# charleschen003/doudizhu-rl

Measured on AMD Instinct MI355X. Metric: env steps/sec (batched tables), higher is better.
Workload: dtype u8; 1 GPU; 65536 tables per GPU, random policy (engine RNG), legal-move list only (no NN), auto-reset: the workload of BASELINE.json configs[1] at the largest single-GPU table count (65,536 per GPU: configs[2] / configs[3]; configs[4] = 8 x 65,536), the same per-GPU workload at every N; tables_per_gpu=65536, total_tables=65536, episodes=2767981, list_layout=slab (fixed-stride segment per table)

## Files before the change

doudizhu-rl_amd/csrc/ddz_engine.hip:

```cpp
#include <hip/hip_runtime.h>
#include <stddef.h>
#include <stdint.h>
#include <stdlib.h>
#include <string.h>

#include <atomic>
#include <mutex>

#include "../../include/ddz_env.h"
#include "ddz_device.h"

using namespace ddz;

namespace {

constexpr int BLOCK = 256;
constexpr int WPB = 16;
constexpr int TB = WPB * 64;
constexpr int STATE_ROW_BYTES = DDZ_NFIELDS * DDZ_ROW;

constexpr int F_ENUM = 1, F_STEP = 2, F_RESET = 4, F_COUNT = 8, F_SLAB = 16;

constexpr int AUTO_SLOTS = 4;
constexpr int AO_HDR_BYTES = 576;
// ... 193 lines not shown
      if (legal) {
        const int64_t pos = o.base + n + pre;
        if (pos < o.cap) {
          o.rows[pos] = row;
          if (IDS) o.ids[pos] = id;
        }
      }
      if (EM == EM_PICK) {
        const int w = pk.want - n;
        if (w >= 0 && w < k) {
          const int src = __builtin_ctzll(__ballot(legal && pre == w));
          pk.r0 = rl(row.x, src); pk.r1 = rl(row.y, src); pk.r2 = rl(row.z, src); pk.r3 = rl(row.w, src);
        }
      }
    }
  }
  return n + k;
}

template <int EM, bool IDS, bool LEAD, class HT>
__device__ __forceinline__ int scan_ids(int id0, int count, const HT& hot, uint64_t hand8, const Follow& f,
                                        int lane, const Out& o, int n, Pick& pk) {
  constexpr bool ROWS = EM == EM_WRITE || EM == EM_PICK;
  constexpr uint64_t H8 = 0x8888888888888888ull;
  const int slot0 = id0 == ID_BIGBANG ? HOT_IDS : id0;
  if (EM == EM_TEAM_PLAN) {
    for (int j0 = 0; j0 < count; j0 += 64, ++pk.rc)
      if (pk.rc < TEAM_ROUNDS)
        pk.desc[pk.rc] = make_uint2(team_x(count - j0, id0 + j0, slot0 + j0), 0u);
    return n;
  }
  for (int j0 = 0; j0 < count; j0 += 64) {
    const int j = j0 + lane;
    const bool in = j < count;
    const int jj = in ? j : 0, id = id0 + jj;
    const uint4 m = hot.meta[slot0 + jj];
    static_assert(!ROWS || HT::HAS_ROWS, "this emission mode reads the unpacked rows");
    const uint4 row = ROWS ? hot.rows[HT::HAS_ROWS ? slot0 + jj : 0] : make_uint4(0, 0, 0, 0);
    const uint64_t nib = (uint64_t)m.x | ((uint64_t)m.y << 32);
    const bool sub = ((hand8 - nib) & H8) == H8;
    const int val = m.z & 0xFF, len = (m.z >> 8) & 0xFF, cat = (m.z >> 16) & 0xFF;
    const bool gate = LEAD || id == 0 || cat == BIGBANG || (cat == QUADRIC && (f.lc != QUADRIC || val > f.lv)) ||
                      (cat == f.lc && f.lc != QUADRIC && len == f.ll && val > f.lv);
    n = scan_emit<EM, IDS>(in && sub && gate, id, nib, cat, (int)(m.z & 0xFFFF), row, o, n, pk);
  }
  return n;
}

template <int EM, bool IDS, class HT>
__device__ __forceinline__ int scan_combos(int list, int count, int idb, uint64_t mainnib, int s, int gap, int mult,
                                           int cat, const HT& hot, uint64_t hand8, int lane, const Out& o,
                                           int n, Pick& pk) {
  constexpr bool ROWS = EM == EM_WRITE || EM == EM_PICK;
  constexpr uint64_t H8 = 0x8888888888888888ull;
  const int L = CL_L[list], off = CL_OFF[list];
  if (EM == EM_TEAM_PLAN) {
    for (int j0 = 0; j0 < count; j0 += 64, ++pk.rc)
      if (pk.rc < TEAM_ROUNDS)
        pk.desc[pk.rc] = make_uint2(team_x(count - j0, idb + j0, off + j0),
                                    1u | (uint32_t)L << 2 | (uint32_t)s << 5 | (uint32_t)gap << 9 | (uint32_t)mult << 12 | (uint32_t)cat << 14);
    return n;
  }
  for (int j0 = 0; j0 < count; j0 += 64) {
    const int j = j0 + lane;
    const bool in = j < count;
    uint64_t nib = mainnib;
    if constexpr (HT::HAS_C64) {
      const uint64_t c = hot.c64[off + (in ? j : 0)], lowm = (1ull << (4 * s)) - 1ull;
      nib += ((c & lowm) | ((c & ~lowm) << (4 * gap))) << (mult - 1);
    } else {
      const uint32_t e = hot.combo[off + (in ? j : 0)];
      for (int k = 0; k < L; ++k) {
        const int pos = (e >> (4 * k)) & 15;
        nib += (uint64_t)mult << (4 * (pos < s ? pos : pos + gap));
      }
    }
    const bool sub = ((hand8 - nib) & H8) == H8;
    const uint4 row = ROWS ? unpack_row(nib, (uint32_t)cat) : make_uint4(0, 0, 0, 0);
    n = scan_emit<EM, IDS>(in && sub, idb + j, nib, cat, s | (gap << 8), row, o, n, pk);
  }
  return n;
}

template <int EM, bool IDS, bool LEAD, class HT>
__device__ __forceinline__ int plan_scan_t(uint64_t hand, const Follow& f, const HT& hot, int lane, const Out& o, Pick& pk) {
  constexpr bool PRUNE = EM != EM_STAGE;
  const uint64_t hand8 = hand | 0x8888888888888888ull;
  const int cnt = lane < 15 ? (int)((hand >> (4 * (lane & 15))) & 15) : 0;
  const uint32_t m1 = (uint32_t)__ballot(cnt >= 1) & M15;
  const uint32_t m2 = (uint32_t)__ballot(cnt >= 2) & M13;
  const uint32_t m3 = (uint32_t)__ballot(cnt >= 3) & M13;
  const uint32_t m4 = (uint32_t)__ballot(cnt >= 4) & M13;
  int n = 0;
  auto scan = [&](int id0, int count) { n = scan_ids<EM, IDS, LEAD>(id0, count, hot, hand8, f, lane, o, n, pk); };
  if (!LEAD && f.lc == BIGBANG) {
    scan(0, 1);
    return n;
  }
  if (LEAD) scan(1, 54); else scan(0, 55);
  const uint32_t above = LEAD ? M15 : gt_mask(f.lv);
  if (LEAD || f.lc == THREE_ONE || f.lc == THREE_TWO) {
    const uint32_t mains = m3 & above;
    if (mains) {
      const int lo = __builtin_ctz(mains), hi = 31 - __builtin_clz(mains);
      if (LEAD || f.lc == THREE_ONE) scan(ID_THREE_ONE + 14 * lo, 14 * (hi - lo + 1));
      if ((LEAD || f.lc == THREE_TWO) && (!PRUNE || __builtin_popcount(m2) >= 2))
        scan(ID_THREE_TWO + 12 * lo, 12 * (hi - lo + 1));
    }
  }
  if (LEAD) {
    const bool a = run_starts(m1 & M12, 5) != 0, b = run_starts(m2 & M12, 3) != 0, c = run_starts(m3 & M12, 2) != 0;
    if (a || b || c) {
      const int lo = a ? ID_SINGLE_LINE : b ? ID_DOUBLE_LINE : ID_TRIPLE_LINE;
      const int hi = c ? ID_THREE_ONE_LINE : b ? ID_TRIPLE_LINE : ID_DOUBLE_LINE;
      scan(lo, hi - lo);
    }
  } else if (f.lc == SINGLE_LINE) {
    scan(ID_SINGLE_LINE, 36);
  } else if (f.lc == DOUBLE_LINE) {
    scan(ID_DOUBLE_LINE, 52);
  } else if (f.lc == TRIPLE_LINE) {
    scan(ID_TRIPLE_LINE, 45);
  }
  auto planes = [&](int cat, int hi, int idb0, int mult, int list2, int list3, int list4, int list5) {
    const uint32_t mm = m3 & M12;
    if (!(LEAD || f.lc == cat)) return;
    for (uint32_t st = mm & (mm >> 1); st; st &= st - 1) {
      const int s = __builtin_ctz(st);
      const int runlen = __builtin_ctz(~(mm >> s));
      int before, sz2, sz3, sz4;
      if (cat == THREE_ONE_LINE) {
        before = 879 * (s < 8 ? s : 8) + (s > 8 ? 627 : 0) + (s > 9 ? 297 : 0);
        sz2 = 77; sz3 = 220; sz4 = 330;
      } else {
        before = 301 * (s < 9 ? s : 9) + (s > 9 ? 175 : 0);
        sz2 = 55; sz3 = 120; sz4 = 126;
      }
      const int maxL = runlen < hi ? runlen : hi;
      for (int L = 2; L <= maxL && s + L <= 12; ++L) {
        if (!(LEAD || (L == f.ll && s > f.lv))) continue;
        if (PRUNE && __builtin_popcount((mult == 1 ? m1 : m2) & ~(((1u << L) - 1u) << s)) < L) continue;
        const int idb = idb0 + before + (L > 2 ? sz2 : 0) + (L > 3 ? sz3 : 0) + (L > 4 ? sz4 : 0);
        const int size = L == 2 ? sz2 : L == 3 ? sz3 : L == 4 ? sz4 : 252;
        const int list = L == 2 ? list2 : L == 3 ? list3 : L == 4 ? list4 : list5;
        const uint64_t mainnib = ((3ull * ONES) & ((1ull << (4 * L)) - 1ull)) << (4 * s);
        n = scan_combos<EM, IDS>(list, size, idb, mainnib, s, L, mult, cat, hot, hand8, lane, o, n, pk);
      }
    }
  };
  planes(THREE_ONE_LINE, 5, ID_THREE_ONE_LINE, 1, 1, 4, 6, 8);
  planes(THREE_TWO_LINE, 4, ID_THREE_TWO_LINE, 2, 3, 5, 7, 7);
  if ((m1 & JOKERS) == JOKERS) scan(ID_BIGBANG, 1);
  if (LEAD || f.lc == FOUR_TAKE_ONE)
    for (uint32_t qm = m4 & above; qm; qm &= qm - 1) {
      const int q = __builtin_ctz(qm);
      n = scan_combos<EM, IDS>(0, 90, ID_FOUR_TAKE_ONE + 90 * q, 4ull << (4 * q), q, 1, 1, FOUR_TAKE_ONE, hot, hand8,
                               lane, o, n, pk);
    }
  if (LEAD || f.lc == FOUR_TAKE_TWO)
    for (uint32_t qm = m4 & above; qm; qm &= qm - 1) {
      const int q = __builtin_ctz(qm);
      if (PRUNE && __builtin_popcount(m2 & ~(1u << q)) < 2) continue;
      n = scan_combos<EM, IDS>(2, 66, ID_FOUR_TAKE_TWO + 66 * q, 4ull << (4 * q), q, 1, 2, FOUR_TAKE_TWO, hot, hand8,
                               lane, o, n, pk);
    }
#if DDZ_NATIVE_JOKER_KICKERS
  if ((m1 & JOKERS) == JOKERS) {
    const uint32_t mm = m3 & M12;
    const uint32_t quads = (LEAD || f.lc == FOUR_TAKE_ONE) ? (m4 & above) : 0u;
    const uint32_t pairs3 = (LEAD || (f.lc == THREE_ONE_LINE && f.ll == 2)) ? (mm & (mm >> 1) & above) : 0u;
    if (EM == EM_TEAM_PLAN) {
      if (quads | pairs3) {
        if (pk.rc < TEAM_ROUNDS) pk.desc[pk.rc] = make_uint2(team_x(24, ID_JK_FOUR, 0), 2u | quads << 2 | pairs3 << 15);
        ++pk.rc;
      }
    } else if (quads | pairs3) {
      const bool isq = lane < 13;
      const int r = isq ? lane : (lane - 13) & 15;
      const bool ok = isq ? ((quads >> r) & 1u) : (lane < 24 && ((pairs3 >> r) & 1u));
      const uint64_t jk = (1ull << 52) | (1ull << 56);
      const uint64_t nib = (isq ? (4ull << (4 * r)) : (0x33ull << (4 * r))) | jk;
      const int cat = isq ? FOUR_TAKE_ONE : THREE_ONE_LINE;
// ... 337 lines not shown
    }
    if (RESET) {
      const uint8_t* mask = (const uint8_t*)a.sel;
      if (!mask || mask[t]) {
        changed = true;
        episode = dealt ? episode + 1 : 0;
        uint64_t h0, h1, h2;
        deal_wave(gid, episode, a.k0, a.k1, lane, h0, h1, h2);
        R = lane == 0 ? unpack_row(h0, 17) : lane == 1 ? unpack_row(h1, 20) : lane == 2 ? unpack_row(h2, 17)
            : lane == DDZ_F_META ? make_uint4(1u | (0xFFu << 16), 1u << 16, episode, 0) : make_uint4(0, 0, 0, 0);
        role = 1; is_done = false; dealt = true;
        qhand = h1; qinfo = mk_info(EMPTY, 0, 1);
      }
    }
    stamps.mark(3);
    if (changed) {
      if (lane < DDZ_NFIELDS) trow[lane] = R;
      if (COUNT || SLAB) {
        hand = qhand;
        info = qinfo;
      }
    }
    if (COUNT) {
      const Out none{nullptr, nullptr, 0, 0, nullptr, nullptr, nullptr};
      Pick nopk{-1, 0, 0, 0, 0};
      const int c = (dealt && !is_done) ? plan_scan<EM_COUNT, false>(hand, info, hot, lane, none, nopk) : 0;
      if (lane == i) new_cnt_l = c;
    }
    if (SLAB) {
      const int64_t sb = t * a.stride;
      const Out o{a.rows, a.ids, sb, sb + a.stride, nullptr, nullptr, nullptr};
      Pick nopk{-1, 0, 0, 0, 0};
      int n = (dealt && !is_done) ? plan_scan<EM_WRITE, IDS>(hand, info, hot, lane, o, nopk) : 0;
      if (n > a.stride) {
        if (lane == 0) atomicOr(a.status, 2);
        n = 0;
      }
      if (lane == 0) a.slab_counts[t] = n;
      slab_rows += n;
    }
    stamps.mark(4);
    base += cnt;
  }
  stamps.set(5, (unsigned long long)ntab);
  stamps.store(t0, lane == 0 && ntab > 0 && SLAB && STEP);
  if (ENUM && ntab > 0 && t0 + ntab == a.T && lane == 0) {
    a.offsets[a.T] = (int32_t)base;
    *a.legal_rows += base;
  }
  if (SLAB && ntab > 0 && lane == 0) {
    int64_t* ws = a.blk_stats + 4 * ((int64_t)blockIdx.x * WPB + wv);
    if (STEP) { ws[0] += s_ply; ws[1] += s_eps; ws[2] += (int64_t)s_lord | ((int64_t)s_up << 32); }
    ws[3] += slab_rows;
  }
  if (COUNT) {
    __shared__ int sh[WPB][4];
    const int incl = wave_incl_scan(new_cnt_l, lane);
    if (lane == 63) {
      sh[wv][0] = incl; sh[wv][1] = s_ply; sh[wv][2] = s_eps; sh[wv][3] = s_lord | (s_up << 16);
    }
    __syncthreads();
    int wbase = 0, tot = 0;
#pragma unroll
    for (int w = 0; w < WPB; ++w) {
      if (w < wv) wbase += sh[w][0];
      tot += sh[w][0];
    }
    if (lane < ntab) {
      a.nxt_counts[t0 + lane] = new_cnt_l;
      a.nxt_local[t0 + lane] = wbase + incl - new_cnt_l;
    }
    if (threadIdx.x == 0) {
      a.nxt_blk[blockIdx.x] = tot;
      if (STEP) {
        int64_t* bs = a.blk_stats + 4 * (int64_t)blockIdx.x;
        int p = 0, e = 0, l = 0, u = 0;
        for (int w = 0; w < WPB; ++w) { p += sh[w][1]; e += sh[w][2]; l += sh[w][3] & 0xFFFF; u += sh[w][3] >> 16; }
        bs[0] += p; bs[1] += e; bs[2] += (int64_t)l | ((int64_t)u << 32);
      }
    }
  }
}

struct RolloutArgs {
  uint8_t* state;
  int64_t T;
  int tpw;
  uint32_t k0, k1;
  uint64_t gid_base;
  int32_t* counts;
  uint4* rows;
  int32_t* ids;
  int64_t stride;
  int64_t it_rows;
  int64_t it_counts;
  int64_t n_iters;
  uint4* traj;
  int64_t* wave_stats;
  int32_t* status;
  int64_t* legal_rows;
};

template <bool IDS, bool TRAJ, bool STAGED = false, int RW = WPB>
__global__ __launch_bounds__(RW * 64, RW == WPB ? 4 : 6) void k_rollout(RolloutArgs a) {
  Stamps<12> stamps;
  __shared__ HotTabT<false> hot;
  __shared__ uint64_t s_stage[RW][STAGE_CAP];
  __shared__ uint16_t s_svl[RW][STAGE_CAP];
  __shared__ uint16_t s_sid[IDS ? RW : 1][IDS ? STAGE_CAP : 1];
  const int lane = threadIdx.x & 63;
  const int wv = (int)rfl(threadIdx.x >> 6);
  const int64_t wave = (int64_t)blockIdx.x * RW + wv;
  const int64_t t0 = wave * a.tpw;
  const int ntab = t0 < a.T ? (int)(a.T - t0 < a.tpw ? a.T - t0 : a.tpw) : 0;
  uint4 Rnext = make_uint4(0, 0, 0, 0);
  if (ntab > 0 && lane < DDZ_NFIELDS) Rnext = ((const uint4*)(a.state + t0 * STATE_ROW_BYTES))[lane];
  hot_fill<RW * 64>(hot);
  __syncthreads();
  uint64_t* stage = s_stage[wv];
  uint16_t* svl = s_svl[wv];
  uint16_t* sid = s_sid[IDS ? wv : 0];
  int s_ply = 0;
  int64_t s_rows = 0;
  const int f_rr = (lane < 16 ? lane - 1 : lane - 16) & 15;
  uint32_t f_bit = lane < 32 ? 1u << lane : 0u;
  uint32_t f_sh = 8u * (uint32_t)(f_rr & 3);
  uint32_t f_w0 = (f_rr >> 2) == 0 ? ~0u : 0u, f_w1 = (f_rr >> 2) == 1 ? ~0u : 0u;
  uint32_t f_w2 = (f_rr >> 2) == 2 ? ~0u : 0u, f_w3 = (f_rr >> 2) == 3 ? ~0u : 0u;
  uint32_t f_grp = (lane >= 1 && lane < 16) ? ~0u : 0u;
  uint32_t f_c4 = (lane >= 16 && lane < 29) ? 4u : 0u;
  uint32_t f_rk = lane == 29 ? (0x00010100u | ((uint32_t)BIGBANG << 24)) : 0u;
  asm volatile("" : "+v"(f_bit), "+v"(f_sh), "+v"(f_w0), "+v"(f_w1), "+v"(f_w2), "+v"(f_w3), "+v"(f_grp), "+v"(f_c4), "+v"(f_rk));
  for (int i = 0; i < ntab; ++i) {
    const int64_t t = t0 + i;
    stamps.mark(0);
    uint4* trow = (uint4*)(a.state + t * STATE_ROW_BYTES);
    const uint4 R = Rnext;
    if (i + 1 < ntab && lane < DDZ_NFIELDS) Rnext = ((const uint4*)(a.state + (t + 1) * STATE_ROW_BYTES))[lane];
    const uint64_t gid = a.gid_base + (uint64_t)t;
    uint64_t P = pack_row(R);
    uint32_t aux = R.w >> 24;
    const uint32_t mx = rl(R.x, DDZ_F_META), my = rl(R.y, DDZ_F_META), mz = rl(R.z, DDZ_F_META);
    const uint32_t my_hi = my & 0xFFFF0000u;
    uint32_t mw = rl(R.w, DDZ_F_META);
    int role = mx & 0xFF;
    if (role > 2) role = 0;
    const bool active = ((my >> 16) & 0xFF) && !((mx >> 8) & 0xFF);
    uint32_t ply = my & 0xFFFF, episode = mz;
    uint64_t hc = rl64(P, DDZ_F_HAND0 + role), hn = rl64(P, DDZ_F_HAND0 + (role == 2 ? 0 : role + 1)),
             hp = rl64(P, DDZ_F_HAND0 + (role == 0 ? 2 : role - 1));
    uint32_t trick = mk_info(EMPTY, 0, 1);
    int passes = 0;
    {
      const int rm1 = role == 0 ? 2 : role - 1, rp1 = role == 2 ? 0 : role + 1;
      const uint64_t n1 = rl64(P, DDZ_F_RECENT0 + rm1), n2 = rl64(P, DDZ_F_RECENT0 + rp1);
      if (n1) trick = info_of_row(n1, (int)rl(aux, DDZ_F_RECENT0 + rm1));
      else if (n2) { trick = info_of_row(n2, (int)rl(aux, DDZ_F_RECENT0 + rp1)); passes = 1; }
    }
    uint32_t draws = 0, dnext = 64;
    uint4* tj = TRAJ ? a.traj + 2 * t : nullptr;
    if (!active) {
      if (lane == 0) {
        a.counts[t] = 0;
        if (STAGED)
          for (int64_t j = 1; j < a.n_iters; ++j) a.counts[t + j * a.it_counts] = 0;
      }
      if (TRAJ) {
        const uint4 f0 = make_uint4(0, 0, 0, 0);
        const uint4 f1 = make_uint4((uint32_t)role | ((mx >> 8) & 0xFF) << 8 | 2u << 24, ply << 16, episode, 0xFFFFFFFFu);
        for (int it = (int)a.n_iters; it > 0; --it) {
          if (lane < 2) tj[lane] = sel4(lane == 0, f0, f1);
          tj += 2 * a.T;
        }
      }
      continue;
    }
    int idle = 0;
    for (int it = (int)a.n_iters; it > 0; --it) {
      uint4 tr0 = make_uint4(0, 0, 0, 0);
      uint4 tr1 = make_uint4((uint32_t)role, ply << 16, episode, 0xFFFFFFFFu);
      if (dnext >= 64u) {
        dnext = 0;
        uint32_t qk0 = a.k0, qk1 = a.k1;
        asm volatile("" : "+s"(qk0), "+s"(qk1));
        draws = philox4x32_10(make_uint4((uint32_t)gid, (uint32_t)(gid >> 32), episode, (2u << 16) | (ply + (uint32_t)lane)), qk0, qk1).x;
      }
      const uint64_t hand = hc;
      const uint32_t info = rfl((passes >= 2) ? mk_info(EMPTY, 0, 1) : trick);
      const int64_t jn = STAGED ? a.n_iters - it : 0;
      const int64_t base = t * a.stride + (STAGED ? jn * a.it_rows : 0);
      int32_t* const cnt_p = a.counts + t + (STAGED ? jn * a.it_counts : 0);
      const uint32_t draw = rl(draws, (int)dnext);
      stamps.mark(1);
      int n = 0, idx = -1;
      uint4 c = make_uint4(0, 0, 0, 0);
      uint64_t snib = 0;
      uint32_t scat = 0, svlv = 0, ncards = 0;
      const int lc0 = (int)(info & 0xFF);
      if (lc0 != EMPTY && lc0 <= TRIPLE) {
        const int lv0 = (int)((info >> 8) & 0xFF);
        const int cntr = lane < 15 ? (int)((hand >> (4 * (lane & 15))) & 15) : 0;
        const uint32_t mlc = (uint32_t)__ballot(cntr >= lc0) & (lc0 == SINGLE ? M15 : M13);
        const uint32_t mq = (uint32_t)__ballot(cntr >= 4) & M13;
        const bool rocket = ((uint32_t)__ballot(cntr >= 1) & JOKERS) == JOKERS;
        const uint32_t ab = gt_mask(lv0);
        const uint32_t cand = mlc & ab;
        const uint32_t bombs = mq;
        const int rr = f_rr;
        const uint32_t okm = 1u | (cand << 1) | (bombs << 16) | (rocket ? 1u << 29 : 0u);
        const bool ok = (okm & f_bit) != 0;
        n = __builtin_popcount(okm);
        const int pre = (int)__builtin_amdgcn_mbcnt_lo(okm, 0u);
        const uint32_t copies = ((uint32_t)lc0 & f_grp) | f_c4;
        const uint32_t dv = copies << f_sh;
        const uint4 row = make_uint4(dv & f_w0, dv & f_w1, dv & f_w2, (dv & f_w3) | (copies << 24) | f_rk);
        if (ok) {
          a.rows[base + pre] = row;
          if (IDS) a.ids[base + pre] = lane == 0 ? 0 : lane < 16 ? (lc0 == SINGLE ? 1 : lc0 == DOUBLE ? 16 : lc0 == TRIPLE ? 29 : 42) + rr
                                      : lane < 29 ? 42 + rr : ID_BIGBANG;
        }
        *cnt_p = n;
        s_rows += n;
        stamps.mark(5);
        idx = (int)__umulhi(draw, (uint32_t)n);
        const int src = __builtin_ctz((uint32_t)__ballot(pre == idx) & okm);
        const int sr = (src < 16 ? src - 1 : src - 16) & 15;
        if (TRAJ) c = make_uint4(rl(row.x, src), rl(row.y, src), rl(row.z, src), rl(row.w, src));
        if (src == 0) { snib = 0; scat = EMPTY; svlv = 1u << 8; }
        else if (src == 29) { snib = (1ull << 52) | (1ull << 56); scat = BIGBANG; svlv = 100u | (1u << 8); ncards = 2; }
        else { scat = src < 16 ? (uint32_t)lc0 : (uint32_t)QUADRIC; snib = (uint64_t)scat << (4 * sr); svlv = (uint32_t)sr | (1u << 8); ncards = scat; }
        stamps.mark(5);
      } else {
        const Out o{nullptr, nullptr, 0, 0, stage, svl, sid};
        Pick pk{-1, 0, 0, 0, 0};
        n = plan_scan<EM_STAGE, IDS>(hand, info, hot, lane, o, pk);
        __builtin_amdgcn_wave_barrier();
        if (n > STAGE_CAP || n > a.stride) {
          if (lane == 0) atomicOr(a.status, 2);
          n = 0;
        }
        stamps.mark(2);
        *cnt_p = n;
        s_rows += n;
        for (int j = lane; j < n; j += 64) {
          const uint64_t e = stage[j];
          a.rows[base + j] = unpack_row(e & 0x0FFFFFFFFFFFFFFFull, (uint32_t)(e >> 60));
          if (IDS) a.ids[base + j] = sid[j];
        }
        stamps.mark(3);
        if (n > 0) {
          idx = (int)__umulhi(draw, (uint32_t)n);
          const uint64_t e = stage[idx];
          const uint64_t anib = e & 0x0FFFFFFFFFFFFFFFull;
          const uint32_t acat = (uint32_t)(e >> 60);
          if (TRAJ) c = unpack_row(anib, acat);
          snib = (uint64_t)rfl((uint32_t)anib) | ((uint64_t)rfl((uint32_t)(anib >> 32)) << 32);
          scat = rfl(acat);
          svlv = rfl((uint32_t)svl[idx]);
          ncards = (uint32_t)nib_sum(snib);
        }
        stamps.mark(10);
      }
      tr1.y |= (uint32_t)n & 0xFFFF;
      if (n <= 0) {
        tr1.x |= 2u << 24;
        idle += 1;
      } else {
        {
          const int d = lane - role;
          const uint64_t add = (d == DDZ_F_HIST0 || lane == DDZ_F_TAKEN) ? snib : 0ull;
          P = d == DDZ_F_RECENT0 ? snib : P + add;
          aux = d == DDZ_F_RECENT0 ? scat : d == DDZ_F_HAND0 ? aux - ncards : aux;
        }
        stamps.mark(6);
        const uint64_t hnew = hand - snib;
        if (snib) { trick = scat | (svlv << 8); passes = 0; } else { passes += 1; }
        const bool won = hnew == 0;
        const uint32_t o_reward = won ? (role == 1 ? 0xFFu : 1u) : 0u;
        tr0 = c;
        tr1.x |= (uint32_t)won << 8 | o_reward << 16;
        tr1.w = (uint32_t)idx;
        ply += 1;
        dnext += 1;
        stamps.mark(7);
        if (won) {
          if (lane == 0) {
            int64_t* ws = a.wave_stats + 4 * wave;
            ws[1] += 1;
            ws[2] += role == 1 ? 1ll : role == 0 ? (1ll << 32) : 0ll;
          }
          episode += 1;
          uint32_t dk0 = a.k0, dk1 = a.k1;
          asm volatile("" : "+s"(dk0), "+s"(dk1));
          uint64_t h0, h1, h2;
#ifdef DDZ_ROLLOUT_DEAL_READLANE
          deal_wave(gid, episode, dk0, dk1, lane, h0, h1, h2);
#else
          deal_wave_lds(gid, episode, dk0, dk1, lane, stage, h0, h1, h2);
#endif
          hc = h1; hn = h2; hp = h0;
          P = 0;
          aux = lane == 1 ? 20u : lane < 3 ? 17u : 0u;
          mw = 0;
          role = 1; ply = 0; trick = mk_info(EMPTY, 0, 1); passes = 0; dnext = 64;
        } else {
          role = role == 2 ? 0 : role + 1;
          hc = hn; hn = hp; hp = hnew;
        }
        stamps.mark(8);
      }
      if (TRAJ && lane < 2) tj[lane] = sel4(lane == 0, tr0, tr1);
      if (TRAJ) tj += 2 * a.T;
      stamps.mark(4);
      __builtin_amdgcn_wave_barrier();
    }
    s_ply += (int)a.n_iters - idle;
    if (idle < (int)a.n_iters) {
      const int rp1 = role == 2 ? 0 : role + 1, rm1 = role == 0 ? 2 : role - 1;
      const uint64_t Pf = lane == role ? hc : lane == rp1 ? hn : lane == rm1 ? hp : P;
      uint4 Rf = unpack_row(Pf, aux);
      if (lane == DDZ_F_META) Rf = make_uint4((uint32_t)role | (0xFFu << 16), ply == 0 ? 1u << 16 : my_hi | (ply & 0xFFFF), episode, mw);
      if (lane < DDZ_NFIELDS) trow[lane] = Rf;
    }
    stamps.mark(9);
  }
  stamps.store(t0, lane == 0 && ntab > 0);
  if (ntab > 0 && lane == 0) {
    int64_t* ws = a.wave_stats + 4 * wave;
    ws[0] += s_ply; ws[3] += s_rows;
  }
}

__device__ __forceinline__ void store_stream(float4* p, const float4 v) {
  __builtin_nontemporal_store(v.x, &p->x);
  __builtin_nontemporal_store(v.y, &p->y);
  __builtin_nontemporal_store(v.z, &p->z);
  __builtin_nontemporal_store(v.w, &p->w);
}

struct SlabArgs {
  uint8_t* state;
  int64_t T;
  int tpw;
  uint32_t k0, k1;
  uint64_t gid_base;
  int auto_reset;
  const void* sel;
  int32_t* counts;
  uint4* rows;
  int32_t* ids;
  int64_t stride;
  uint8_t* done;
  int8_t* reward;
  uint8_t* illegal;
  uint4* traj;
  int64_t* wave_stats;
  int32_t* status;
  uint64_t thr;
  int32_t* choice_out;
  float4* face;
  int face_variant;
  int coop;
  int team;
  int lpt;
};
constexpr int STEP_Q = 4;

struct FastLanes {
  int rr;
  uint32_t bit, sh, w0, w1, w2, w3, grp, c4, rk;
};
__device__ __forceinline__ FastLanes fast_lanes(int lane) {
  FastLanes f;
  f.rr = (lane < 16 ? lane - 1 : lane - 16) & 15;
  f.bit = lane < 32 ? 1u << lane : 0u;
  f.sh = 8u * (uint32_t)(f.rr & 3);
  f.w0 = (f.rr >> 2) == 0 ? ~0u : 0u; f.w1 = (f.rr >> 2) == 1 ? ~0u : 0u;
  f.w2 = (f.rr >> 2) == 2 ? ~0u : 0u; f.w3 = (f.rr >> 2) == 3 ? ~0u : 0u;
  f.grp = (lane >= 1 && lane < 16) ? ~0u : 0u;
  f.c4 = (lane >= 16 && lane < 29) ? 4u : 0u;
  f.rk = lane == 29 ? (0x00010100u | ((uint32_t)BIGBANG << 24)) : 0u;
  asm volatile("" : "+v"(f.bit), "+v"(f.sh), "+v"(f.w0), "+v"(f.w1), "+v"(f.w2), "+v"(f.w3), "+v"(f.grp), "+v"(f.c4), "+v"(f.rk));
  return f;
}

template <bool IDS, class HT>
__device__ __forceinline__ int slab_list(uint64_t hand, uint32_t info, int64_t base, int64_t stride, uint4* rows, int32_t* ids,
                                         const HT& hot, int lane, const FastLanes& fl, int32_t* status) {
  const int lc0 = (int)(info & 0xFF);
  int n;
  if (hand != 0 && lc0 != EMPTY && lc0 <= TRIPLE && !(info & (QF_FROZEN | QF_BADLAST))) {
    const int lv0 = (int)((info >> 8) & 0xFF);
    const int cntr = lane < 15 ? (int)((hand >> (4 * (lane & 15))) & 15) : 0;
    const uint32_t mlc = (uint32_t)__ballot(cntr >= lc0) & (lc0 == SINGLE ? M15 : M13);
    const uint32_t mq = (uint32_t)__ballot(cntr >= 4) & M13;
    const bool rocket = ((uint32_t)__ballot(cntr >= 1) & JOKERS) == JOKERS;
    const uint32_t okm = 1u | ((mlc & gt_mask(lv0)) << 1) | (mq << 16) | (rocket ? 1u << 29 : 0u);
    n = __builtin_popcount(okm);
    const int pre = (int)__builtin_amdgcn_mbcnt_lo(okm, 0u);
    const uint32_t copies = ((uint32_t)lc0 & fl.grp) | fl.c4;
    const uint32_t dv = copies << fl.sh;
    const uint4 row = make_uint4(dv & fl.w0, dv & fl.w1, dv & fl.w2, (dv & fl.w3) | (copies << 24) | fl.rk);
    if ((okm & fl.bit) != 0) {
      rows[base + pre] = row;
      if (IDS) ids[base + pre] = lane == 0 ? 0 : lane < 16 ? (lc0 == SINGLE ? 1 : lc0 == DOUBLE ? 16 : 29) + fl.rr
                                 : lane < 29 ? 42 + fl.rr : ID_BIGBANG;
    }
  } else {
    const Out o{rows, ids, base, base + stride, nullptr, nullptr, nullptr};
    Pick pk{-1, 0, 0, 0, 0};
    n = plan_scan<EM_SLAB, IDS>(hand, info, hot, lane, o, pk);
    if (n > stride) {
      if (lane == 0 && status) atomicOr(status, 2);
      n = 0;
    }
  }
  return n;
}

template <bool WRITE, bool IDS, class HT>
__device__ __forceinline__ int team_round(uint2 d, uint64_t hand8, const HT& hot, int lane, int64_t base, int64_t cap, uint4* rows,
                                          int32_t* ids) {
  constexpr uint64_t H8 = 0x8888888888888888ull;
  const uint32_t dx = rfl(d.x), dy = rfl(d.y);
  const int nv = (int)(dx & 63u) + 1, id = (int)((dx >> 6) & 0x3FFFu) + lane, so = (int)(dx >> 20);
  const bool in = lane < nv;
  const uint32_t kind = dy & 3u;
  uint64_t nib;
  int cat;
  bool ok = in;
  if (kind == 0) {
    const uint4 m = hot.meta[so + (in ? lane : 0)];
    nib = (uint64_t)m.x | ((uint64_t)m.y << 32);
    cat = (int)((m.z >> 16) & 0xFF);
  } else if (kind == 1) {
    const int L = (int)((dy >> 2) & 7u), s_ = (int)((dy >> 5) & 15u), gap = (int)((dy >> 9) & 7u);
    const int mult = (int)((dy >> 12) & 3u);
    cat = (int)((dy >> 14) & 31u);
    const uint64_t unit = (cat == FOUR_TAKE_ONE || cat == FOUR_TAKE_TWO) ? 4ull : 3ull;
    nib = ((unit * ONES) & ((1ull << (4 * gap)) - 1ull)) << (4 * s_);
    if constexpr (HT::HAS_C64) {
      const uint64_t c = hot.c64[so + (in ? lane : 0)], lowm = (1ull << (4 * s_)) - 1ull;
      nib += ((c & lowm) | ((c & ~lowm) << (4 * gap))) << (mult - 1);
    } else {
      const uint32_t e = hot.combo[so + (in ? lane : 0)];
      for (int k = 0; k < L; ++k) {
        const int pos = (int)((e >> (4 * k)) & 15u);
        nib += (uint64_t)mult << (4 * (pos < s_ ? pos : pos + gap));
      }
    }
  } else {
    const uint32_t quads = (dy >> 2) & 0x1FFFu, pairs3 = dy >> 15;
    const bool isq = lane < 13;
    const int r = isq ? lane : (lane - 13) & 15;
    ok = isq ? ((quads >> r) & 1u) : (lane < 24 && ((pairs3 >> r) & 1u));
    nib = (isq ? (4ull << (4 * r)) : (0x33ull << (4 * r))) | (1ull << 52) | (1ull << 56);
    cat = isq ? FOUR_TAKE_ONE : THREE_ONE_LINE;
  }
  const bool legal = ok && ((hand8 - nib) & H8) == H8;
  const uint64_t bl = __ballot(legal);
  if (WRITE && legal) {
    const int pre = __builtin_amdgcn_mbcnt_hi((uint32_t)(bl >> 32), __builtin_amdgcn_mbcnt_lo((uint32_t)bl, 0u));
    const int64_t pos = base + pre;
    if (pos < cap) {
      rows[pos] = unpack_row(nib, (uint32_t)cat);
      if (IDS) ids[pos] = id;
    }
// ... 2337 lines not shown
```

Measured before the change: 4.633 billion env steps/s.

## Emit base single/pair/triple/bomb moves directly from ballots, skipping staged scan when no tail

In the rollout kernel, the lead and non-simple follow cases now build the base move set (singles, pairs, triples, bombs, rocket) directly from lane ballot masks and write rows straight to the slab. The staged hot-table scan runs only when tail combos such as lines or three-with-kickers are possible, and then it only covers the remaining ids through a new BASE template flag. The common case avoids LDS staging and the table scan, at the cost of more branching and code size. Move ordering has to match the previous id ordering for the outputs to stay identical.

New measurement: 4.778 billion env steps/s (median of 6 runs). +3.1%, better.

```diff
diff --git a/doudizhu-rl_amd/csrc/ddz_engine.hip b/doudizhu-rl_amd/csrc/ddz_engine.hip
--- a/doudizhu-rl_amd/csrc/ddz_engine.hip
+++ b/doudizhu-rl_amd/csrc/ddz_engine.hip
@@ -299,7 +299,7 @@
   return n;
 }
 
-template <int EM, bool IDS, bool LEAD, class HT>
+template <int EM, bool IDS, bool LEAD, class HT, bool BASE = true>
 __device__ __forceinline__ int plan_scan_t(uint64_t hand, const Follow& f, const HT& hot, int lane, const Out& o, Pick& pk) {
   constexpr bool PRUNE = EM != EM_STAGE;
   const uint64_t hand8 = hand | 0x8888888888888888ull;
@@ -311,10 +311,12 @@
   int n = 0;
   auto scan = [&](int id0, int count) { n = scan_ids<EM, IDS, LEAD>(id0, count, hot, hand8, f, lane, o, n, pk); };
   if (!LEAD && f.lc == BIGBANG) {
-    scan(0, 1);
+    if (BASE) scan(0, 1);
     return n;
   }
-  if (LEAD) scan(1, 54); else scan(0, 55);
+  if (BASE) {
+    if (LEAD) scan(1, 54); else scan(0, 55);
+  }
   const uint32_t above = LEAD ? M15 : gt_mask(f.lv);
   if (LEAD || f.lc == THREE_ONE || f.lc == THREE_TWO) {
     const uint32_t mains = m3 & above;
@@ -818,6 +820,98 @@
   }
 }
 
+struct FastLanes {
+  static constexpr bool WIDE = false;
+  int rr;
+  uint32_t bit, sh, w0, w1, w2, w3, grp, c4, rk;
+};
+__device__ __forceinline__ FastLanes fast_lanes(int lane) {
+  FastLanes f;
+  f.rr = (lane < 16 ? lane - 1 : lane - 16) & 15;
+  f.bit = lane < 32 ? 1u << lane : 0u;
+  f.sh = 8u * (uint32_t)(f.rr & 3);
+  f.w0 = (f.rr >> 2) == 0 ? ~0u : 0u; f.w1 = (f.rr >> 2) == 1 ? ~0u : 0u;
+  f.w2 = (f.rr >> 2) == 2 ? ~0u : 0u; f.w3 = (f.rr >> 2) == 3 ? ~0u : 0u;
+  f.grp = (lane >= 1 && lane < 16) ? ~0u : 0u;
+  f.c4 = (lane >= 16 && lane < 29) ? 4u : 0u;
+  f.rk = lane == 29 ? (0x00010100u | ((uint32_t)BIGBANG << 24)) : 0u;
+  asm volatile("" : "+v"(f.bit), "+v"(f.sh), "+v"(f.w0), "+v"(f.w1), "+v"(f.w2), "+v"(f.w3), "+v"(f.grp), "+v"(f.c4), "+v"(f.rk));
+  return f;
+}
+struct LeadLanes {
+  static constexpr bool WIDE = true;
+  int rr;
+  uint32_t copies, sh, w0, w1, w2, w3, rk;
+};
+__device__ __forceinline__ LeadLanes lead_lanes(int lane) {
+  LeadLanes f;
+  const int g = (lane >= 15) + (lane >= 28) + (lane >= 41);
+  f.rr = lane < 54 ? lane - (g ? 2 + 13 * g : 0) : 0;
+  f.copies = lane < 54 ? (uint32_t)g + 1u : 0u;
+  f.sh = 8u * (uint32_t)(f.rr & 3);
+  f.w0 = (f.rr >> 2) == 0 ? ~0u : 0u; f.w1 = (f.rr >> 2) == 1 ? ~0u : 0u;
+  f.w2 = (f.rr >> 2) == 2 ? ~0u : 0u; f.w3 = (f.rr >> 2) == 3 ? ~0u : 0u;
+  f.rk = lane == 54 ? (0x00010100u | ((uint32_t)BIGBANG << 24)) : 0u;
+  return f;
+}
+__device__ __forceinline__ int round_pre(uint32_t okm) { return (int)__builtin_amdgcn_mbcnt_lo(okm, 0u); }
+__device__ __forceinline__ int round_pre(uint64_t okm) {
+  return (int)__builtin_amdgcn_mbcnt_hi((uint32_t)(okm >> 32), __builtin_amdgcn_mbcnt_lo((uint32_t)okm, 0u));
+}
+template <bool IDS, class L, class M>
+__device__ __forceinline__ int round_emit(M okm, const L& ln, uint32_t copies, int id, uint4* rows, int32_t* ids, int64_t pos0,
+                                          uint4& row, int& pre) {
+  static_assert(L::WIDE == (sizeof(M) == 8), "the lead layout has 55 lanes");
+  int n;
+  bool ok;
+  pre = round_pre(okm);
+  if constexpr (L::WIDE) {
+    n = __builtin_popcountll(okm);
+    ok = ((okm >> (threadIdx.x & 63)) & 1ull) != 0;
+  } else {
+    n = __builtin_popcount(okm);
+    ok = (okm & ln.bit) != 0;
+  }
+  const uint32_t dv = copies << ln.sh;
+  row = make_uint4(dv & ln.w0, dv & ln.w1, dv & ln.w2, (dv & ln.w3) | (copies << 24) | ln.rk);
+  if (ok) {
+    rows[pos0 + pre] = row;
+    if (IDS) ids[pos0 + pre] = id;
+  }
+  return n;
+}
+template <bool WIDE, class M>
+__device__ __forceinline__ int round_src(M okm, int pre, int idx) {
+  if constexpr (WIDE) return __builtin_ctzll(__ballot(pre == idx) & okm);
+  else return __builtin_ctz((uint32_t)__ballot(pre == idx) & okm);
+}
+template <bool WIDE>
+__device__ __forceinline__ void round_entry(int src, uint32_t gsz, uint64_t& snib, uint32_t& scat, uint32_t& svlv, uint32_t& ncards) {
+  if (src == (WIDE ? 54 : 29)) {
+    snib = (1ull << 52) | (1ull << 56); scat = BIGBANG; svlv = 100u | (1u << 8); ncards = 2;
+  } else if (!WIDE && src == 0) {
+    snib = 0; scat = EMPTY; svlv = 1u << 8; ncards = 0;
+  } else {
+    int sr;
+    if constexpr (WIDE) {
+      const int g = (src >= 15) + (src >= 28) + (src >= 41);
+      sr = src - (g ? 2 + 13 * g : 0);
+      scat = (uint32_t)g + 1u;
+    } else {
+      sr = (src < 16 ? src - 1 : src - 16) & 15;
+      scat = src < 16 ? gsz : (uint32_t)QUADRIC;
+    }
+    snib = (uint64_t)scat << (4 * sr); svlv = (uint32_t)sr | (1u << 8); ncards = scat;
+  }
+}
+template <bool TRAJ, bool WIDE, class M>
+__device__ __forceinline__ void round_pick(M okm, int pre, const uint4& row, int idx, uint32_t gsz, uint4& c, uint64_t& snib,
+                                           uint32_t& scat, uint32_t& svlv, uint32_t& ncards) {
+  const int src = round_src<WIDE>(okm, pre, idx);
+  if (TRAJ) c = make_uint4(rl(row.x, src), rl(row.y, src), rl(row.z, src), rl(row.w, src));
+  round_entry<WIDE>(src, gsz, snib, scat, svlv, ncards);
+}
+
 struct RolloutArgs {
   uint8_t* state;
   int64_t T;
@@ -858,15 +952,7 @@
   uint16_t* sid = s_sid[IDS ? wv : 0];
   int s_ply = 0;
   int64_t s_rows = 0;
-  const int f_rr = (lane < 16 ? lane - 1 : lane - 16) & 15;
-  uint32_t f_bit = lane < 32 ? 1u << lane : 0u;
-  uint32_t f_sh = 8u * (uint32_t)(f_rr & 3);
-  uint32_t f_w0 = (f_rr >> 2) == 0 ? ~0u : 0u, f_w1 = (f_rr >> 2) == 1 ? ~0u : 0u;
-  uint32_t f_w2 = (f_rr >> 2) == 2 ? ~0u : 0u, f_w3 = (f_rr >> 2) == 3 ? ~0u : 0u;
-  uint32_t f_grp = (lane >= 1 && lane < 16) ? ~0u : 0u;
-  uint32_t f_c4 = (lane >= 16 && lane < 29) ? 4u : 0u;
-  uint32_t f_rk = lane == 29 ? (0x00010100u | ((uint32_t)BIGBANG << 24)) : 0u;
-  asm volatile("" : "+v"(f_bit), "+v"(f_sh), "+v"(f_w0), "+v"(f_w1), "+v"(f_w2), "+v"(f_w3), "+v"(f_grp), "+v"(f_c4), "+v"(f_rk));
+  const FastLanes fl = fast_lanes(lane);
   for (int i = 0; i < ntab; ++i) {
     const int64_t t = t0 + i;
     stamps.mark(0);
@@ -933,69 +1019,107 @@
       uint64_t snib = 0;
       uint32_t scat = 0, svlv = 0, ncards = 0;
       const int lc0 = (int)(info & 0xFF);
+      const int cntr = lane < 15 ? (int)((hand >> (4 * (lane & 15))) & 15) : 0;
+      uint4 row = make_uint4(0, 0, 0, 0);
+      int pre = 0;
+      auto whole = [&](int n0) {
+        n = n0;
+        *cnt_p = n;
+        s_rows += n;
+        idx = (int)__umulhi(draw, (uint32_t)n);
+      };
+      const int fid = !IDS ? 0 : lane == 0 ? 0 : lane < 16 ? (lc0 == SINGLE ? 1 : lc0 == DOUBLE ? 16 : lc0 == TRIPLE ? 29 : 42) + fl.rr
+                                 : lane < 29 ? 42 + fl.rr : ID_BIGBANG;
       if (lc0 != EMPTY && lc0 <= TRIPLE) {
         const int lv0 = (int)((info >> 8) & 0xFF);
-        const int cntr = lane < 15 ? (int)((hand >> (4 * (lane & 15))) & 15) : 0;
         const uint32_t mlc = (uint32_t)__ballot(cntr >= lc0) & (lc0 == SINGLE ? M15 : M13);
         const uint32_t mq = (uint32_t)__ballot(cntr >= 4) & M13;
         const bool rocket = ((uint32_t)__ballot(cntr >= 1) & JOKERS) == JOKERS;
-        const uint32_t ab = gt_mask(lv0);
-        const uint32_t cand = mlc & ab;
-        const uint32_t bombs = mq;
-        const int rr = f_rr;
-        const uint32_t okm = 1u | (cand << 1) | (bombs << 16) | (rocket ? 1u << 29 : 0u);
-        const bool ok = (okm & f_bit) != 0;
-        n = __builtin_popcount(okm);
-        const int pre = (int)__builtin_amdgcn_mbcnt_lo(okm, 0u);
-        const uint32_t copies = ((uint32_t)lc0 & f_grp) | f_c4;
-        const uint32_t dv = copies << f_sh;
-        const uint4 row = make_uint4(dv & f_w0, dv & f_w1, dv & f_w2, (dv & f_w3) | (copies << 24) | f_rk);
-        if (ok) {
-          a.rows[base + pre] = row;
-          if (IDS) a.ids[base + pre] = lane == 0 ? 0 : lane < 16 ? (lc0 == SINGLE ? 1 : lc0 == DOUBLE ? 16 : lc0 == TRIPLE ? 29 : 42) + rr
-                                      : lane < 29 ? 42 + rr : ID_BIGBANG;
-        }
-        *cnt_p = n;
-        s_rows += n;
-        stamps.mark(5);
-        idx = (int)__umulhi(draw, (uint32_t)n);
-        const int src = __builtin_ctz((uint32_t)__ballot(pre == idx) & okm);
-        const int sr = (src < 16 ? src - 1 : src - 16) & 15;
-        if (TRAJ) c = make_uint4(rl(row.x, src), rl(row.y, src), rl(row.z, src), rl(row.w, src));
-        if (src == 0) { snib = 0; scat = EMPTY; svlv = 1u << 8; }
-        else if (src == 29) { snib = (1ull << 52) | (1ull << 56); scat = BIGBANG; svlv = 100u | (1u << 8); ncards = 2; }
-        else { scat = src < 16 ? (uint32_t)lc0 : (uint32_t)QUADRIC; snib = (uint64_t)scat << (4 * sr); svlv = (uint32_t)sr | (1u << 8); ncards = scat; }
+        const uint32_t okm = 1u | ((mlc & gt_mask(lv0)) << 1) | (mq << 16) | (rocket ? 1u << 29 : 0u);
+        const uint32_t copies = ((uint32_t)lc0 & fl.grp) | fl.c4;
+        whole(round_emit<IDS>(okm, fl, copies, fid, a.rows, a.ids, base, row, pre));
+        round_pick<TRAJ, false>(okm, pre, row, idx, (uint32_t)lc0, c, snib, scat, svlv, ncards);
         stamps.mark(5);
       } else {
-        const Out o{nullptr, nullptr, 0, 0, stage, svl, sid};
-        Pick pk{-1, 0, 0, 0, 0};
-        n = plan_scan<EM_STAGE, IDS>(hand, info, hot, lane, o, pk);
-        __builtin_amdgcn_wave_barrier();
-        if (n > STAGE_CAP || n > a.stride) {
-          if (lane == 0) atomicOr(a.status, 2);
-          n = 0;
+        const uint32_t m1 = (uint32_t)__ballot(cntr >= 1) & M15, m2 = (uint32_t)__ballot(cntr >= 2) & M13;
+        const uint32_t m3 = (uint32_t)__ballot(cntr >= 3) & M13, m4 = (uint32_t)__ballot(cntr >= 4) & M13;
+        const bool jokers = (m1 & JOKERS) == JOKERS;
+        const bool lead = lc0 == EMPTY;
+        uint64_t okm;
+        bool tail;
+        int n0;
+        if (lead) {
+          tail = m3 != 0 || run_starts(m1 & M12, 5) != 0 || run_starts(m2 & M12, 3) != 0 || m1 == 0;
+          okm = (uint64_t)m1 | (uint64_t)m2 << 15 | (uint64_t)m3 << 28 | (uint64_t)m4 << 41 |
+                (jokers && !tail ? 1ull << 54 : 0ull);
+          int ln = lane;
+          asm volatile("" : "+v"(ln));
+          const LeadLanes ll = lead_lanes(ln);
+          n0 = round_emit<IDS>(okm, ll, ll.copies, ln < 54 ? 1 + ln : ID_BIGBANG, a.rows, a.ids, base, row, pre);
+        } else {
+          const int lv0 = (int)((info >> 8) & 0xFF), ll0 = (int)((info >> 16) & 0xFF);
+          const uint32_t ab = gt_mask(lv0);
+          uint32_t cand = 0, bombs = m4, may = 0;
+          bool rocket = jokers;
+          if (lc0 == QUADRIC) { cand = m4 & ab; bombs = 0; }
+          else if (lc0 == BIGBANG) { bombs = 0; rocket = false; }
+          else if (lc0 == THREE_ONE || lc0 == THREE_TWO) may = m3 & ab;
+          else if (lc0 == SINGLE_LINE) may = run_starts(m1 & M12, ll0) & ab;
+          else if (lc0 == DOUBLE_LINE) may = run_starts(m2 & M12, ll0) & ab;
+          else if (lc0 == TRIPLE_LINE || lc0 == THREE_ONE_LINE || lc0 == THREE_TWO_LINE) may = run_starts(m3 & M12, ll0) & ab;
+          else if (lc0 == FOUR_TAKE_ONE || lc0 == FOUR_TAKE_TWO) may = m4 & ab;
+          tail = may != 0 || m1 == 0;
+          const uint32_t okf = m1 == 0 ? 0u : 1u | (cand << 1) | (bombs << 16) | (rocket && !tail ? 1u << 29 : 0u);
+          const uint32_t copies = ((uint32_t)lc0 & fl.grp) | fl.c4;
+          n0 = round_emit<IDS>(okf, fl, copies, fid, a.rows, a.ids, base, row, pre);
+          okm = okf;
         }
-        stamps.mark(2);
-        *cnt_p = n;
-        s_rows += n;
-        for (int j = lane; j < n; j += 64) {
-          const uint64_t e = stage[j];
-          a.rows[base + j] = unpack_row(e & 0x0FFFFFFFFFFFFFFFull, (uint32_t)(e >> 60));
-          if (IDS) a.ids[base + j] = sid[j];
+        if (!tail) {
+          whole(n0);
+          if (lead) round_pick<TRAJ, true>(okm, pre, row, idx, 0u, c, snib, scat, svlv, ncards);
+          else round_pick<TRAJ, false>((uint32_t)okm, pre, row, idx, (uint32_t)lc0, c, snib, scat, svlv, ncards);
+          stamps.mark(11);
+        } else {
+          const Out o{nullptr, nullptr, 0, 0, stage, svl, sid};
+          Pick pk{-1, 0, 0, 0, 0};
+          const Follow f = follow_of(info);
+          const int n1 = lead ? plan_scan_t<EM_STAGE, IDS, true, HotTabT<false>, false>(hand, f, hot, lane, o, pk)
+                              : plan_scan_t<EM_STAGE, IDS, false, HotTabT<false>, false>(hand, f, hot, lane, o, pk);
+          __builtin_amdgcn_wave_barrier();
+          n = n0 + n1;
+          if (n > STAGE_CAP || n > a.stride) {
+            if (lane == 0) atomicOr(a.status, 2);
+            n = 0;
+          }
+          stamps.mark(2);
+          *cnt_p = n;
+          s_rows += n;
+          const int64_t tbase = base + n0;
+          for (int j = lane; j < n - n0; j += 64) {
+            const uint64_t e = stage[j];
+            a.rows[tbase + j] = unpack_row(e & 0x0FFFFFFFFFFFFFFFull, (uint32_t)(e >> 60));
+            if (IDS) a.ids[tbase + j] = sid[j];
+          }
+          stamps.mark(3);
+          if (n > 0) {
+            idx = (int)__umulhi(draw, (uint32_t)n);
+            if (idx < n0) {
+              if (lead) round_entry<true>(round_src<true>(okm, round_pre(okm), idx), 0u, snib, scat, svlv, ncards);
+              else round_entry<false>(round_src<false>((uint32_t)okm, round_pre((uint32_t)okm), idx), (uint32_t)lc0, snib, scat, svlv, ncards);
+              if (TRAJ) c = unpack_row(snib, scat);
+            } else {
+              const uint64_t e = stage[idx - n0];
+              const uint64_t anib = e & 0x0FFFFFFFFFFFFFFFull;
+              const uint32_t acat = (uint32_t)(e >> 60);
+              if (TRAJ) c = unpack_row(anib, acat);
+              snib = (uint64_t)rfl((uint32_t)anib) | ((uint64_t)rfl((uint32_t)(anib >> 32)) << 32);
+              scat = rfl(acat);
+              svlv = rfl((uint32_t)svl[idx - n0]);
+              ncards = (uint32_t)nib_sum(snib);
+            }
+          }
+          stamps.mark(10);
         }
-        stamps.mark(3);
-        if (n > 0) {
-          idx = (int)__umulhi(draw, (uint32_t)n);
-          const uint64_t e = stage[idx];
-          const uint64_t anib = e & 0x0FFFFFFFFFFFFFFFull;
-          const uint32_t acat = (uint32_t)(e >> 60);
-          if (TRAJ) c = unpack_row(anib, acat);
-          snib = (uint64_t)rfl((uint32_t)anib) | ((uint64_t)rfl((uint32_t)(anib >> 32)) << 32);
-          scat = rfl(acat);
-          svlv = rfl((uint32_t)svl[idx]);
-          ncards = (uint32_t)nib_sum(snib);
-        }
-        stamps.mark(10);
       }
       tr1.y |= (uint32_t)n & 0xFFFF;
       if (n <= 0) {
@@ -1101,24 +1225,6 @@
   int lpt;
 };
 constexpr int STEP_Q = 4;
-
-struct FastLanes {
-  int rr;
-  uint32_t bit, sh, w0, w1, w2, w3, grp, c4, rk;
-};
-__device__ __forceinline__ FastLanes fast_lanes(int lane) {
-  FastLanes f;
-  f.rr = (lane < 16 ? lane - 1 : lane - 16) & 15;
-  f.bit = lane < 32 ? 1u << lane : 0u;
-  f.sh = 8u * (uint32_t)(f.rr & 3);
-  f.w0 = (f.rr >> 2) == 0 ? ~0u : 0u; f.w1 = (f.rr >> 2) == 1 ? ~0u : 0u;
-  f.w2 = (f.rr >> 2) == 2 ? ~0u : 0u; f.w3 = (f.rr >> 2) == 3 ? ~0u : 0u;
-  f.grp = (lane >= 1 && lane < 16) ? ~0u : 0u;
-  f.c4 = (lane >= 16 && lane < 29) ? 4u : 0u;
-  f.rk = lane == 29 ? (0x00010100u | ((uint32_t)BIGBANG << 24)) : 0u;
-  asm volatile("" : "+v"(f.bit), "+v"(f.sh), "+v"(f.w0), "+v"(f.w1), "+v"(f.w2), "+v"(f.w3), "+v"(f.grp), "+v"(f.c4), "+v"(f.rk));
-  return f;
-}
 
 template <bool IDS, class HT>
 __device__ __forceinline__ int slab_list(uint64_t hand, uint32_t info, int64_t base, int64_t stride, uint4* rows, int32_t* ids,
```
